# JuanDuGit/DH3D

Measured on AMD Instinct MI355X. Metric: point-clouds/sec, higher is better.
Workload: dtype f32; 1 GPU; local-descriptor forward (basic_config), N=8192 K=8, batch=8; clouds_per_gpu=8, clouds_total=8, points=8192, knn=8, parallelism=clouds sharded over 1 GPU(s), no data-path collective, weights=random-init (no checkpoint blobs exist upstream), steps_in_flight=4

## Files before the change

dh3d_amd/csrc/knn.hip:

```cpp
#include <float.h>
#include <limits.h>

#include <type_traits>

#include "common.h"
#include "wave_ops.h"

#pragma clang fp contract(off)

namespace {

typedef float f32x2 __attribute__((ext_vector_type(2)));
typedef unsigned long long u64;

constexpr int kQueriesPerBlock = 256;
constexpr int kChunk = 1024;
constexpr int kQueue = 16;

struct KnnLadder {
  int log2ct;
  int ctmask;
  int cv;
};

static KnnLadder knn_ladder(int N) {
  int t, v;
  if (N <= 32) { t = 32; v = 1; }
  else if (N <= 64) { t = 64; v = 1; }
  else if (N <= 128) { t = 128; v = 1; }
  else if (N <= 256) { t = 128; v = 2; }
  else if (N <= 512) { t = 128; v = 4; }
  else if (N <= 1024) { t = 256; v = 4; }
  else if (N <= 2048) { t = 256; v = 8; }
  else if (N <= 4096) { t = 512; v = 8; }
  else if (N <= 8192) { t = 1024; v = 8; }
  else { t = 1024; v = (N + 1023) / 1024; }
  KnnLadder l;
  l.ctmask = t - 1;
  l.cv = v;
  l.log2ct = 0;
  while ((1 << l.log2ct) < t) ++l.log2ct;
  return l;
}

__device__ __forceinline__ int cand_slot(int c, int comp) {
  const int g = c >> 2, r = c & 3;
  const int off = (r < 2) ? (2 * comp + r) : (4 + 2 * comp + r);
  return g * 12 + off;
}

__device__ __forceinline__ float knn_bcast(float v, int lane) {
  return __int_as_float(__builtin_amdgcn_readlane(__float_as_int(v), lane));
}

__device__ __forceinline__ int knn_pick_near(unsigned long long m, int gl) {
  const unsigned long long up = m >> gl, dn = m & ((1ull << gl) - 1);
  const int da = up ? __builtin_ctzll(up) : 128;
  const int db = dn ? gl - (63 - __builtin_clzll(dn)) : 128;
  return da <= db ? gl + da : gl - db;
}

template <int KMAX>
struct KnnState {
  u64 keys[KMAX];
  float bound;
};

template <int KMAX, bool KEEP_MIN = false>
__device__ __forceinline__ void knn_insert_key(KnnState<KMAX> &st, const u64 key) {
  if (key < st.keys[KMAX - 1]) {
    if constexpr (KMAX <= 16) {
      bool lt[KMAX];
#pragma unroll
      for (int i = 0; i < KMAX - 1; ++i) lt[i] = key < st.keys[i];
      lt[KMAX - 1] = true;
#pragma unroll
      for (int i = KMAX - 1; i > 0; --i) {
        const u64 in = lt[i - 1] ? st.keys[i - 1] : key;
        st.keys[i] = lt[i] ? in : st.keys[i];
      }
      st.keys[0] = lt[0] ? key : st.keys[0];
    } else {
      st.keys[KMAX - 1] = key;
#pragma unroll
      for (int i = KMAX - 1; i > 0; --i) {
        const u64 a = st.keys[i - 1], b = st.keys[i];
        const bool lt = b < a;
        st.keys[i - 1] = lt ? b : a;
        st.keys[i] = lt ? a : b;
      }
    }
    const unsigned hb = (unsigned)(st.keys[KMAX - 1] >> 32);
    if (hb <= 0x7f800000u) {
      const float dk = __uint_as_float(hb);
      const float nb = __fmul_rn(__fmul_rn(dk, dk), 1.000001f);
      st.bound = KEEP_MIN ? fminf(st.bound, nb) : nb;
    }
  }
}
template <int KMAX, bool KEEP_MIN = false>
__device__ __forceinline__ void knn_offer(KnnState<KMAX> &st, float s, int x, const KnnLadder &lad) {
  if (s <= st.bound) {
    const float d = sqrtf(s);
    const unsigned tb = (unsigned)((x & lad.ctmask) * lad.cv + (x >> lad.log2ct));
    knn_insert_key<KMAX, KEEP_MIN>(st, ((u64)__float_as_uint(d) << 32) | tb);
  }
}


__device__ __forceinline__ void knn_dist8(const float *g0, const f32x2 qx2, const f32x2 qy2, const f32x2 qz2,
                                          f32x2 (&s)[4]) {
  const f32x4 a0 = *reinterpret_cast<const f32x4 *>(g0), a1 = *reinterpret_cast<const f32x4 *>(g0 + 4),
              a2 = *reinterpret_cast<const f32x4 *>(g0 + 8), b0 = *reinterpret_cast<const f32x4 *>(g0 + 12),
              b1 = *reinterpret_cast<const f32x4 *>(g0 + 16), b2 = *reinterpret_cast<const f32x4 *>(g0 + 20);
  {
    const f32x2 dx = f32x2{a0[0], a0[1]} - qx2, dy = f32x2{a0[2], a0[3]} - qy2, dz = f32x2{a1[0], a1[1]} - qz2;
    s[0] = __builtin_elementwise_fma(dz, dz, __builtin_elementwise_fma(dy, dy, dx * dx));
  }
  {
    const f32x2 dx = f32x2{a1[2], a1[3]} - qx2, dy = f32x2{a2[0], a2[1]} - qy2, dz = f32x2{a2[2], a2[3]} - qz2;
    s[1] = __builtin_elementwise_fma(dz, dz, __builtin_elementwise_fma(dy, dy, dx * dx));
  }
  {
    const f32x2 dx = f32x2{b0[0], b0[1]} - qx2, dy = f32x2{b0[2], b0[3]} - qy2, dz = f32x2{b1[0], b1[1]} - qz2;
    s[2] = __builtin_elementwise_fma(dz, dz, __builtin_elementwise_fma(dy, dy, dx * dx));
  }
  {
    const f32x2 dx = f32x2{b1[2], b1[3]} - qx2, dy = f32x2{b2[0], b2[1]} - qy2, dz = f32x2{b2[2], b2[3]} - qz2;
    s[3] = __builtin_elementwise_fma(dz, dz, __builtin_elementwise_fma(dy, dy, dx * dx));
  }
}
__device__ __forceinline__ float knn_min8(const f32x2 (&s)[4]) {
  return fminf(fminf(fminf(s[0][0], s[0][1]), fminf(s[1][0], s[1][1])),
               fminf(fminf(s[2][0], s[2][1]), fminf(s[3][0], s[3][1])));
}

template <int KMAX, bool XYZ_LAYOUT>
__global__ __launch_bounds__(kQueriesPerBlock) void knn_kernel(const float *__restrict__ pos, int N,
                                                              int K, KnnLadder lad,
                                                              int32_t *__restrict__ nn,
                                                              float *__restrict__ dist) {
  __shared__ __attribute__((aligned(16))) float s_c[kChunk * 3];
  __shared__ uint2 s_q[kQueue * kQueriesPerBlock];
  const int b = blockIdx.y;
  const int tid = threadIdx.x;
  const int y = blockIdx.x * kQueriesPerBlock + tid;
  const float *pc = pos + (size_t)b * 3 * N;

  float qx = 0.f, qy = 0.f, qz = 0.f;
  if (y < N) {
    if (XYZ_LAYOUT) { qx = pc[(size_t)y * 3]; qy = pc[(size_t)y * 3 + 1]; qz = pc[(size_t)y * 3 + 2]; }
    else { qx = pc[y]; qy = pc[(size_t)N + y]; qz = pc[(size_t)2 * N + y]; }
  }
  const f32x2 qx2 = {qx, qx}, qy2 = {qy, qy}, qz2 = {qz, qz};

  KnnState<KMAX> st;
#pragma unroll
  for (int i = 0; i < KMAX; ++i) st.keys[i] = ~0ull;
  st.bound = INFINITY;
  int cnt = 0;

  for (int base = 0; base < N; base += kChunk) {
    const int len = min(kChunk, N - base);
    const int len8 = (len + 31) & ~31;
    __syncthreads();
    if (XYZ_LAYOUT) {
      for (int e = tid; e < len8 * 3; e += kQueriesPerBlock) {
        const int c = e / 3, comp = e - c * 3;
        s_c[cand_slot(c, comp)] = c < len ? pc[(size_t)base * 3 + e] : INFINITY;
      }
    } else {
      for (int e = tid; e < len8 * 3; e += kQueriesPerBlock) {
        const int comp = e / len8, c = e - comp * len8;
        s_c[cand_slot(c, comp)] = c < len ? pc[(size_t)comp * N + base + c] : INFINITY;
      }
    }
    __syncthreads();
    const int len32 = (len8 + 31) & ~31;
    for (int j = 0; j < len32; j += 32) {
      f32x2 s[4][4];
      float mn[4];
#pragma unroll
      for (int u = 0; u < 4; ++u) {
        knn_dist8(s_c + ((j >> 2) + 2 * u) * 12, qx2, qy2, qz2, s[u]);
        mn[u] = knn_min8(s[u]);
      }
      const float m = fminf(fminf(mn[0], mn[1]), fminf(mn[2], mn[3]));
      if (__any(y < N && m <= st.bound)) {
#pragma unroll
        for (int u = 0; u < 4; ++u) {
          if (y < N && mn[u] <= st.bound) {
#pragma unroll
            for (int t = 0; t < 8; ++t) {
              const float sv = s[u][t >> 1][t & 1];
              const int x = base + j + 8 * u + t;
              if (sv <= st.bound && x < N) {
                s_q[cnt * kQueriesPerBlock + tid] = make_uint2(__float_as_uint(sv), (unsigned)x);
                ++cnt;
              }
            }
          }
          if (__any(cnt > kQueue - 8)) {
            for (int i = 0; i < kQueue; ++i) {
              if (!__any(i < cnt)) break;
              if (i < cnt) {
                const uint2 e = s_q[i * kQueriesPerBlock + tid];
                knn_offer<KMAX>(st, __uint_as_float(e.x), (int)e.y, lad);
              }
            }
            cnt = 0;
          }
        }
      }
    }
  }
  for (int i = 0; i < kQueue; ++i) {
    if (i < cnt) {
      const uint2 e = s_q[i * kQueriesPerBlock + tid];
      knn_offer<KMAX>(st, __uint_as_float(e.x), (int)e.y, lad);
    }
  }

  if (y < N) {
    int32_t *o_nn = nn + ((size_t)b * N + y) * K;
    float *o_d = dist + ((size_t)b * N + y) * K;
#pragma unroll
    for (int i = 0; i < KMAX; ++i) {
      if (i < K) {
        const unsigned tb = (unsigned)st.keys[i];
        if (st.keys[i] == ~0ull) {
          o_nn[i] = -1;
          o_d[i] = FLT_MAX;
        } else {
          o_nn[i] = (int)(((tb % (unsigned)lad.cv) << lad.log2ct) + tb / (unsigned)lad.cv);
          o_d[i] = __uint_as_float((unsigned)(st.keys[i] >> 32));
        }
      }
    }
  }
}

constexpr int kSortedWaves = 4;
constexpr int kCellInts = 4112;
constexpr int kCellFlag = 4106;

template <int KMAX>
__global__ __launch_bounds__(64 * kSortedWaves) void knn_sorted_kernel(const float4 *__restrict__ sorted,
                                                                    const float *__restrict__ gbox, int N,
                                                                    int K, KnnLadder lad,
                                                                    int32_t *__restrict__ nn,
                                                                    float *__restrict__ dist, const int *__restrict__ gate) {
  if (gate && !gate[(size_t)blockIdx.y * kCellInts + kCellFlag]) return;
  __shared__ __attribute__((aligned(16))) float s_c[kSortedWaves][64 * 3];
  __shared__ uint2 s_q[kSortedWaves][kQueue * 64];
  __shared__ int s_id[kSortedWaves][64];
  const int b = blockIdx.y;
  const int lane = threadIdx.x & 63, wave = threadIdx.x >> 6;
  const int NG = (N + 63) / 64;
  const int g = blockIdx.x * kSortedWaves + wave;
  if (g >= NG) return;
  const float4 *sc = sorted + (size_t)b * N;
  const float4 *gb = reinterpret_cast<const float4 *>(gbox) + (size_t)b * NG * 2;
  float *my_c = s_c[wave];
  uint2 *my_q = s_q[wave];
  int *my_id = s_id[wave];

  const int qi = g * 64 + lane;
  const bool valid = qi < N;
  const float4 pad = make_float4(INFINITY, INFINITY, INFINITY, __int_as_float(-1));
  float4 qr = valid ? sc[qi] : pad;
  const f32x2 qx2 = {qr.x, qr.x}, qy2 = {qr.y, qr.y}, qz2 = {qr.z, qr.z};
  const float4 qlo = gb[g * 2], qhi = gb[g * 2 + 1];

  KnnState<KMAX> st;
#pragma unroll
  for (int i = 0; i < KMAX; ++i) st.keys[i] = ~0ull;
  st.bound = INFINITY;
  int cnt = 0;
  float wave_bound = INFINITY;

  auto drain = [&]() {
    const int deepest = -wave_min_i32(-cnt);
    uint2 nxt = my_q[lane];
#pragma unroll 1
    for (int i = 0; i < deepest; ++i) {
      const uint2 e = nxt;
      if (i + 1 < deepest) nxt = my_q[(i + 1) * 64 + lane];
      if (i < cnt) knn_offer<KMAX>(st, __uint_as_float(e.x), (int)e.y, lad);
    }
    cnt = 0;
    wave_bound = wave_max_f32(valid ? st.bound : 0.f);
  };

  auto scan_group = [&](int gcc, const float4 cr) {
    my_c[cand_slot(lane, 0)] = cr.x;
    my_c[cand_slot(lane, 1)] = cr.y;
    my_c[cand_slot(lane, 2)] = cr.z;
    my_id[lane] = __float_as_int(cr.w);
    __builtin_amdgcn_wave_barrier();
    const int clen = min(64, N - gcc * 64);
    for (int j = 0; j < clen; j += 32) {
      f32x2 s[4][4];
      float mn[4];
#pragma unroll
      for (int u = 0; u < 4; ++u) {
        knn_dist8(my_c + ((j >> 2) + 2 * u) * 12, qx2, qy2, qz2, s[u]);
        mn[u] = knn_min8(s[u]);
      }
      const float m = fminf(fminf(mn[0], mn[1]), fminf(mn[2], mn[3]));
      if (__any(valid && m <= st.bound)) {
#pragma unroll
        for (int u = 0; u < 4; ++u) {
          if (valid && mn[u] <= st.bound) {
#pragma unroll
            for (int t = 0; t < 8; ++t) {
              const float sv = s[u][t >> 1][t & 1];
              if (sv <= st.bound && j + 8 * u + t < clen) {
                my_q[cnt * 64 + lane] = make_uint2(__float_as_uint(sv), (unsigned)my_id[j + 8 * u + t]);
                ++cnt;
              }
            }
          }
          if (__any(cnt > kQueue - 8)) drain();
        }
      }
    }
    __builtin_amdgcn_wave_barrier();
  };
  auto load_group = [&](int gcc) { const int ci = gcc * 64 + lane; return ci < N ? sc[ci] : pad; };

  scan_group(g, qr);
  if (__any(cnt > 0)) drain();

  const int cg = g >> 6, NC = (NG + 63) >> 6;
  for (int tier = 0; tier < 2; ++tier) {
    for (int k = 0; k < 2 * NC; ++k) {
      const int ci = cg + ((k & 1) ? (k + 1) / 2 : -(k / 2));
      if (ci < 0 || ci >= NC) continue;
      const int c0 = ci * 64, gl = min(max(g - c0, 0), 63);
      const int gi = c0 + lane;
      const bool other = gi < NG && gi != g;
      float bd = INFINITY;
      float4 clo = make_float4(INFINITY, INFINITY, INFINITY, 0.f), chi = clo;
      if (other) {
        clo = gb[gi * 2];
        chi = gb[gi * 2 + 1];
        const float ex = fmaxf(fmaxf(clo.x - qhi.x, qlo.x - chi.x), 0.f);
        const float ey = fmaxf(fmaxf(clo.y - qhi.y, qlo.y - chi.y), 0.f);
        const float ez = fmaxf(fmaxf(clo.z - qhi.z, qlo.z - chi.z), 0.f);
        bd = (ex * ex + ey * ey + ez * ez) * 0.99999f;
      }
      unsigned long long mask =
          tier == 0 ? __ballot(other && bd == 0.f) : __ballot(other && bd > 0.f && bd <= wave_bound);
      if (!mask) continue;
      int l = knn_pick_near(mask, gl);
      mask &= ~(1ull << l);
      float4 nxt = load_group(c0 + l);
      while (true) {
        const int lcur = l;
        const float4 cr = nxt;
        const bool more = mask != 0;
        if (more) {
          l = knn_pick_near(mask, gl);
          mask &= ~(1ull << l);
          nxt = load_group(c0 + l);
        }
        const float bdl = __int_as_float(__builtin_amdgcn_readlane(__float_as_int(bd), lcur));
        if (bdl <= wave_bound) {
          const float lx = knn_bcast(clo.x, lcur), ly = knn_bcast(clo.y, lcur), lz = knn_bcast(clo.z, lcur);
          const float hx = knn_bcast(chi.x, lcur), hy = knn_bcast(chi.y, lcur), hz = knn_bcast(chi.z, lcur);
          const float px = fmaxf(fmaxf(lx - qr.x, qr.x - hx), 0.f);
          const float py = fmaxf(fmaxf(ly - qr.y, qr.y - hy), 0.f);
          const float pz = fmaxf(fmaxf(lz - qr.z, qr.z - hz), 0.f);
          const float pd = (px * px + py * py + pz * pz) * 0.99999f;
          if (__any(valid && pd <= st.bound)) scan_group(c0 + lcur, cr);
        }
        if (!more) break;
      }
    }
  }
  if (__any(cnt > 0)) drain();

  if (valid) {
    const int y = __float_as_int(qr.w);
    int32_t *o_nn = nn + ((size_t)b * N + y) * K;
    float *o_d = dist + ((size_t)b * N + y) * K;
#pragma unroll
    for (int i = 0; i < KMAX; ++i) {
      if (i < K) {
        const unsigned tb = (unsigned)st.keys[i];
        if (st.keys[i] == ~0ull) {
          o_nn[i] = -1;
          o_d[i] = FLT_MAX;
        } else {
          o_nn[i] = (int)(((tb % (unsigned)lad.cv) << lad.log2ct) + tb / (unsigned)lad.cv);
          o_d[i] = __uint_as_float((unsigned)(st.keys[i] >> 32));
        }
      }
    }
  }
}

template <int S>
__host__ __device__ constexpr int knn_split_lds_bytes() {
  return S * (64 * 3 * 4 + kQueue * 64 * 8 + 64 * 4 + 64 * 4 + 64 * 4);
}
template <int KMAX, int S>
__device__ __forceinline__ void knn_split_body(const float4 *__restrict__ sorted, const float *__restrict__ gbox, int N, int K,
                                               const KnnLadder lad, int32_t *__restrict__ nn, float *__restrict__ dist,
                                               const int b, const int g, unsigned char *lds, const int wave0 = 0) {
  static_assert(KMAX * 64 * sizeof(u64) <= kQueue * 64 * sizeof(uint2), "a K-list fits its wave's survivor queue");
  uint2 (*s_q)[kQueue * 64] = reinterpret_cast<uint2 (*)[kQueue * 64]>(lds);
  float (*s_c)[64 * 3] = reinterpret_cast<float (*)[64 * 3]>(lds + S * kQueue * 64 * 8);
  int (*s_id)[64] = reinterpret_cast<int (*)[64]>(lds + S * (kQueue * 64 * 8 + 64 * 3 * 4));
  float (*s_share)[64] = reinterpret_cast<float (*)[64]>(lds + S * (kQueue * 64 * 8 + 64 * 3 * 4 + 64 * 4));
  float (*s_kth)[64] = reinterpret_cast<float (*)[64]>(lds + S * (kQueue * 64 * 8 + 64 * 3 * 4 + 64 * 8));
  constexpr int R = (KMAX + S - 1) / S - 1;
  const int lane = threadIdx.x & 63;
  const int wave = __builtin_amdgcn_readfirstlane((int)(threadIdx.x >> 6) - wave0);
  const int NG = (N + 63) / 64;
  const float4 *sc = sorted + (size_t)b * N;
  const float4 *gb = reinterpret_cast<const float4 *>(gbox) + (size_t)b * NG * 2;
  float *my_c = s_c[wave];
  uint2 *my_q = s_q[wave];
  int *my_id = s_id[wave];

  const int qi = g * 64 + lane;
  const bool valid = qi < N;
  const float4 pad = make_float4(INFINITY, INFINITY, INFINITY, __int_as_float(-1));
  const float4 qr = valid ? sc[qi] : pad;
  const f32x2 qx2 = {qr.x, qr.x}, qy2 = {qr.y, qr.y}, qz2 = {qr.z, qr.z};
  const float4 qlo = gb[g * 2], qhi = gb[g * 2 + 1];

  KnnState<KMAX> st;
#pragma unroll
  for (int i = 0; i < KMAX; ++i) st.keys[i] = ~0ull;
  st.bound = INFINITY;
  int cnt = 0;
  float wave_bound = INFINITY;
  s_share[wave][lane] = INFINITY;
  s_kth[wave][lane] = INFINITY;
  __syncthreads();

  auto adopt = [&](float mx) {
    float mk = st.bound;
#pragma unroll
    for (int w = 1; w < S; ++w) {
      mx = fmaxf(mx, s_share[(wave + w) % S][lane]);
      mk = fminf(mk, s_kth[(wave + w) % S][lane]);
    }
    st.bound = fminf(mk, mx);
    wave_bound = wave_max_f32(valid ? st.bound : 0.f);
  };

  auto drain = [&]() {
    const int deepest = -wave_min_i32(-cnt);
    uint2 nxt = my_q[lane];
#pragma unroll 1
    for (int i = 0; i < deepest; ++i) {
      const uint2 e = nxt;
      if (i + 1 < deepest) nxt = my_q[(i + 1) * 64 + lane];
      if (i < cnt) knn_offer<KMAX, true>(st, __uint_as_float(e.x), (int)e.y, lad);
    }
    cnt = 0;
    const unsigned hb = (unsigned)(st.keys[R] >> 32);
    float mx = INFINITY;
    if (hb <= 0x7f800000u) {
      const float dr = __uint_as_float(hb);
      mx = __fmul_rn(__fmul_rn(dr, dr), 1.000001f);
    }
    s_share[wave][lane] = mx;
    const unsigned hk = (unsigned)(st.keys[KMAX - 1] >> 32);
    if (hk <= 0x7f800000u) {
      const float dk = __uint_as_float(hk);
      s_kth[wave][lane] = __fmul_rn(__fmul_rn(dk, dk), 1.000001f);
    }
    adopt(mx);
  };

  auto scan_group = [&](int gcc, const float4 cr) {
    my_c[cand_slot(lane, 0)] = cr.x;
    my_c[cand_slot(lane, 1)] = cr.y;
    my_c[cand_slot(lane, 2)] = cr.z;
    my_id[lane] = __float_as_int(cr.w);
    __builtin_amdgcn_wave_barrier();
    const int clen = min(64, N - gcc * 64);
    for (int j = 0; j < clen; j += 32) {
      f32x2 sq[4][4];
      float mn[4];
#pragma unroll
      for (int u = 0; u < 4; ++u) {
        knn_dist8(my_c + ((j >> 2) + 2 * u) * 12, qx2, qy2, qz2, sq[u]);
        mn[u] = knn_min8(sq[u]);
      }
      const float m = fminf(fminf(mn[0], mn[1]), fminf(mn[2], mn[3]));
      if (__any(valid && m <= st.bound)) {
#pragma unroll
        for (int u = 0; u < 4; ++u) {
          if (valid && mn[u] <= st.bound) {
#pragma unroll
            for (int t = 0; t < 8; ++t) {
              const float sv = sq[u][t >> 1][t & 1];
              if (sv <= st.bound && j + 8 * u + t < clen) {
                my_q[cnt * 64 + lane] = make_uint2(__float_as_uint(sv), (unsigned)my_id[j + 8 * u + t]);
                ++cnt;
              }
            }
          }
          if (__any(cnt > kQueue - 8)) drain();
        }
      }
    }
    __builtin_amdgcn_wave_barrier();
  };
  auto load_group = [&](int gcc) { const int ci = gcc * 64 + lane; return ci < N ? sc[ci] : pad; };

  const int NO = (NG - wave + S - 1) / S, NCH = (NO + 63) >> 6;
  const int jg = g / S, cj = min(jg >> 6, max(NCH - 1, 0));
  bool other = false;
  float bd = INFINITY;
  float4 clo = make_float4(INFINITY, INFINITY, INFINITY, 0.f), chi = clo;
  auto fetch_boxes = [&](int ci) {
    const int j = ci * 64 + lane, gi = j * S + wave;
    other = j < NO && gi != g;
    if (other) {
      clo = gb[gi * 2];
      chi = gb[gi * 2 + 1];
    }
  };
  auto test_boxes = [&]() {
    bd = INFINITY;
    if (other) {
      const float ex = fmaxf(fmaxf(clo.x - qhi.x, qlo.x - chi.x), 0.f);
      const float ey = fmaxf(fmaxf(clo.y - qhi.y, qlo.y - chi.y), 0.f);
      const float ez = fmaxf(fmaxf(clo.z - qhi.z, qlo.z - chi.z), 0.f);
      bd = (ex * ex + ey * ey + ez * ez) * 0.99999f;
    }
  };
  if (NCH == 1) fetch_boxes(0);

  {
    my_c[cand_slot(lane, 0)] = qr.x;
    my_c[cand_slot(lane, 1)] = qr.y;
    my_c[cand_slot(lane, 2)] = qr.z;
    my_id[lane] = __float_as_int(qr.w);
    __builtin_amdgcn_wave_barrier();
    const int clen = min(64, N - g * 64);
    for (int blk = wave; blk * 8 < clen; blk += S) {
      f32x2 sq[4];
      knn_dist8(my_c + 2 * blk * 12, qx2, qy2, qz2, sq);
      if (valid) {
#pragma unroll
        for (int t = 0; t < 8; ++t) {
          const float sv = sq[t >> 1][t & 1];
          if (sv <= st.bound && blk * 8 + t < clen) {
            my_q[cnt * 64 + lane] = make_uint2(__float_as_uint(sv), (unsigned)my_id[blk * 8 + t]);
            ++cnt;
          }
        }
      }
      if (__any(cnt > 0)) drain();
    }
    __builtin_amdgcn_wave_barrier();
    __syncthreads();
    adopt(s_share[wave][lane]);
  }
  for (int tier = 0; tier < 2; ++tier) {
    for (int k = 0; k < 2 * NCH; ++k) {
      const int ci = cj + ((k & 1) ? (k + 1) / 2 : -(k / 2));
      if (ci < 0 || ci >= NCH) continue;
      if (NCH > 1) fetch_boxes(ci);
      if (NCH > 1 || tier == 0) test_boxes();
      const int gl = min(max(jg - ci * 64, 0), 63);
      if (tier == 1) adopt(s_share[wave][lane]);
      unsigned long long mask =
          tier == 0 ? __ballot(other && bd == 0.f) : __ballot(other && bd > 0.f && bd <= wave_bound);
      if (!mask) continue;
      int l = knn_pick_near(mask, gl);
      mask &= ~(1ull << l);
      float4 nxt = load_group((ci * 64 + l) * S + wave);
      while (true) {
        const int lcur = l;
        const float4 cr = nxt;
        const bool more = mask != 0;
        if (more) {
          l = knn_pick_near(mask, gl);
          mask &= ~(1ull << l);
          nxt = load_group((ci * 64 + l) * S + wave);
        }
        const float bdl = knn_bcast(bd, lcur);
        if (bdl <= wave_bound) {
          const float lx = knn_bcast(clo.x, lcur), ly = knn_bcast(clo.y, lcur), lz = knn_bcast(clo.z, lcur);
          const float hx = knn_bcast(chi.x, lcur), hy = knn_bcast(chi.y, lcur), hz = knn_bcast(chi.z, lcur);
          const float px = fmaxf(fmaxf(lx - qr.x, qr.x - hx), 0.f);
          const float py = fmaxf(fmaxf(ly - qr.y, qr.y - hy), 0.f);
          const float pz = fmaxf(fmaxf(lz - qr.z, qr.z - hz), 0.f);
          const float pd = (px * px + py * py + pz * pz) * 0.99999f;
          if (__any(valid && pd <= st.bound)) scan_group((ci * 64 + lcur) * S + wave, cr);
        }
        if (!more) break;
      }
    }
  }
  if (__any(cnt > 0)) drain();

  for (int step = S / 2; step >= 1; step >>= 1) {
    __syncthreads();
    if (wave >= step && wave < 2 * step) {
#pragma unroll
      for (int i = 0; i < KMAX; ++i)
        my_q[i * 64 + lane] = make_uint2((unsigned)st.keys[i], (unsigned)(st.keys[i] >> 32));
    }
    __syncthreads();
    if (wave < step) {
      const uint2 *oq = s_q[wave + step];
#pragma unroll
      for (int i = 0; i < KMAX; ++i) {
        const uint2 e = oq[i * 64 + lane];
        const u64 key = ((u64)e.y << 32) | e.x;
        if (key < st.keys[KMAX - 1]) {
          st.keys[KMAX - 1] = key;
#pragma unroll
          for (int t = KMAX - 1; t > 0; --t) {
            const u64 a = st.keys[t - 1], c = st.keys[t];
            const bool lt = c < a;
            st.keys[t - 1] = lt ? c : a;
            st.keys[t] = lt ? a : c;
          }
        }
      }
    }
  }

  if (wave == 0 && valid) {
    const int y = __float_as_int(qr.w);
    int32_t *o_nn = nn + ((size_t)b * N + y) * K;
    float *o_d = dist + ((size_t)b * N + y) * K;
#pragma unroll
    for (int i = 0; i < KMAX; ++i) {
      if (i < K) {
        const unsigned tb = (unsigned)st.keys[i];
        if (st.keys[i] == ~0ull) {
          o_nn[i] = -1;
          o_d[i] = FLT_MAX;
        } else {
          o_nn[i] = (int)(((tb % (unsigned)lad.cv) << lad.log2ct) + tb / (unsigned)lad.cv);
          o_d[i] = __uint_as_float((unsigned)(st.keys[i] >> 32));
        }
      }
    }
  }
}


template <int KMAX, int S>
__global__ __launch_bounds__(64 * S) void knn_split_kernel(const float4 *__restrict__ sorted,
                                                         const float *__restrict__ gbox, int N, int K,
                                                         KnnLadder lad, int32_t *__restrict__ nn,
                                                         float *__restrict__ dist, const int *__restrict__ gate) {
  if (gate && !gate[(size_t)blockIdx.y * kCellInts + kCellFlag]) return;
  __shared__ __attribute__((aligned(16))) unsigned char s_lds[knn_split_lds_bytes<S>()];
  const unsigned ng = (unsigned)((N + 63) / 64);
  knn_split_body<KMAX, S>(sorted, gbox, N, K, lad, nn, dist, blockIdx.y, (int)((blockIdx.x + 37u * blockIdx.y) % ng), s_lds);
}

template <int CPL, bool XYZ>
__global__ __launch_bounds__(256) void knn_small_kernel(const float *__restrict__ pos, int N, int K, KnnLadder lad,
                                                       int32_t *__restrict__ nn, float *__restrict__ dist, int Q) {
  const int b = blockIdx.y, lane = threadIdx.x & 63;
  const int wave = __builtin_amdgcn_readfirstlane(threadIdx.x >> 6);
  const int q0 = (blockIdx.x * 4 + wave) * Q;
  if (q0 >= N) return;
  const float *base = pos + (size_t)b * N * 3;
  float cx[CPL], cy[CPL], cz[CPL];
  unsigned tbk[CPL];
#pragma unroll
  for (int c = 0; c < CPL; ++c) {
    const int j = lane + 64 * c, jj = j < N ? j : 0;
    cx[c] = XYZ ? base[(size_t)jj * 3] : base[jj];
    cy[c] = XYZ ? base[(size_t)jj * 3 + 1] : base[(size_t)N + jj];
    cz[c] = XYZ ? base[(size_t)jj * 3 + 2] : base[(size_t)2 * N + jj];
    tbk[c] = j < N ? (unsigned)((j & lad.ctmask) * lad.cv + (j >> lad.log2ct)) : 0xFFFFFFFFu;
  }
#pragma unroll 1
  for (int qi = 0; qi < Q; ++qi) {
    const int q = q0 + qi;
    if (q >= N) break;
    const float qx = XYZ ? base[(size_t)q * 3] : base[q];
    const float qy = XYZ ? base[(size_t)q * 3 + 1] : base[(size_t)N + q];
    const float qz = XYZ ? base[(size_t)q * 3 + 2] : base[(size_t)2 * N + q];
    unsigned kd[CPL];
#pragma unroll
    for (int c = 0; c < CPL; ++c) {
      const float dx = qx - cx[c], dy = qy - cy[c], dz = qz - cz[c];
      const float d = sqrtf(__builtin_fmaf(dz, dz, __builtin_fmaf(dy, dy, dx * dx)));
      kd[c] = tbk[c] != 0xFFFFFFFFu ? __float_as_uint(d) : 0xFFFFFFFFu;
    }
    u64 need = 0;
    unsigned my_hi = 0xFFFFFFFFu, my_lo = 0xFFFFFFFFu;
    u64 m1 = ~0ull, m2 = ~0ull;
    bool more = false;
    auto rescan = [&]() {
      m1 = ~0ull; m2 = ~0ull;
      int cnt = 0;
#pragma unroll
      for (int c = 0; c < CPL; ++c) {
        const u64 key = ((u64)kd[c] << 32) | tbk[c];
        const bool ok = key >= need && key != ~0ull;
        const bool c1 = ok && key < m1, c2 = ok && key < m2;
        m2 = c1 ? m1 : (c2 ? key : m2);
        m1 = c1 ? key : m1;
        cnt += ok ? 1 : 0;
      }
      more = cnt > 2;
    };
    rescan();
    for (int r = 0; r < K; ++r) {
      const unsigned hi = wave_min_u32((unsigned)(m1 >> 32));
      const unsigned lo = wave_min_u32((unsigned)(m1 >> 32) == hi ? (unsigned)m1 : 0xFFFFFFFFu);
      if (lane == r) { my_hi = hi; my_lo = lo; }
      const u64 sel = ((u64)hi << 32) | lo;
      if (sel == ~0ull) break;
      need = sel + 1;
      const bool won = m1 == sel;
      const bool dry = won && m2 == ~0ull && more;
      m1 = won ? m2 : m1;
      m2 = won ? ~0ull : m2;
      if (__ballot(dry) != 0ull) rescan();
    }
    if (lane < K) {
      const size_t o = ((size_t)b * N + q) * K + lane;
      if (my_hi == 0xFFFFFFFFu && my_lo == 0xFFFFFFFFu) {
        nn[o] = -1;
        dist[o] = FLT_MAX;
      } else {
        nn[o] = (int)(((my_lo % (unsigned)lad.cv) << lad.log2ct) + my_lo / (unsigned)lad.cv);
        dist[o] = __uint_as_float(my_hi);
      }
    }
  }
}

template <bool XYZ>
int knn_launch(const float *pos, int B, int N, int K, int32_t *nn, float *dist, hipStream_t s) {
  const KnnLadder lad = knn_ladder(N);
  if (N <= 2048) {
    const int Q = (long long)B * N <= 16384 ? 2 : 4;
    dim3 sgrid(dh3d_cdiv(N, 4 * Q), B), sblock(256);
    if (N <= 512) hipLaunchKernelGGL((knn_small_kernel<8, XYZ>), sgrid, sblock, 0, s, pos, N, K, lad, nn, dist, Q);
    else if (N <= 1024) hipLaunchKernelGGL((knn_small_kernel<16, XYZ>), sgrid, sblock, 0, s, pos, N, K, lad, nn, dist, Q);
    else hipLaunchKernelGGL((knn_small_kernel<32, XYZ>), sgrid, sblock, 0, s, pos, N, K, lad, nn, dist, Q);
    return dh3d_launch_status();
  }
  dim3 grid(dh3d_cdiv(N, kQueriesPerBlock), B), block(kQueriesPerBlock);
  if (K <= 4) hipLaunchKernelGGL((knn_kernel<4, XYZ>), grid, block, 0, s, pos, N, K, lad, nn, dist);
  else if (K <= 8) hipLaunchKernelGGL((knn_kernel<8, XYZ>), grid, block, 0, s, pos, N, K, lad, nn, dist);
  else if (K <= 16) hipLaunchKernelGGL((knn_kernel<16, XYZ>), grid, block, 0, s, pos, N, K, lad, nn, dist);
  else if (K <= 32) hipLaunchKernelGGL((knn_kernel<32, XYZ>), grid, block, 0, s, pos, N, K, lad, nn, dist);
  else hipLaunchKernelGGL((knn_kernel<64, XYZ>), grid, block, 0, s, pos, N, K, lad, nn, dist);
  return dh3d_launch_status();
}

template <int KMAX>
__global__ __launch_bounds__(256) void knn_anydp_kernel(const float *__restrict__ pos, int Dp, int N, int K, KnnLadder lad,
                                                        int32_t *__restrict__ nn, float *__restrict__ dist) {
  __shared__ float s_c[16][256];
  const int b = blockIdx.y, y = blockIdx.x * 256 + threadIdx.x;
  const float *pc = pos + (size_t)b * Dp * N;
  float q[16];
#pragma unroll
  for (int dp = 0; dp < 16; ++dp) q[dp] = (dp < Dp && y < N) ? pc[(size_t)dp * N + y] : 0.f;
  u64 keys[KMAX];
#pragma unroll
  for (int i = 0; i < KMAX; ++i) keys[i] = ~0ull;
  for (int x0 = 0; x0 < N; x0 += 256) {
    __syncthreads();
    for (int dp = 0; dp < Dp; ++dp) s_c[dp][threadIdx.x] = x0 + (int)threadIdx.x < N ? pc[(size_t)dp * N + x0 + threadIdx.x] : 0.f;
    __syncthreads();
    const int cnt = min(256, N - x0);
    for (int j = 0; j < cnt; ++j) {
      float sum = 0.f;
      for (int dp = 0; dp < Dp; ++dp) {
        const float val = s_c[dp][j] - q[dp];
        sum = __builtin_fmaf(val, val, sum);
      }
      const float d = sqrtf(sum);
      const int x = x0 + j;
      const unsigned tb = (unsigned)((x & lad.ctmask) * lad.cv + (x >> lad.log2ct));
      const u64 key = ((u64)__float_as_uint(d) << 32) | tb;
      if (key < keys[K - 1]) {
        int i = K - 1;
        while (i > 0 && keys[i - 1] > key) { keys[i] = keys[i - 1]; --i; }
        keys[i] = key;
      }
    }
  }
  if (y >= N) return;
  int32_t *o_nn = nn + ((size_t)b * N + y) * K;
  float *o_d = dist + ((size_t)b * N + y) * K;
  for (int i = 0; i < K; ++i) {
    if (keys[i] == ~0ull) { o_nn[i] = -1; o_d[i] = 3.402823466e+38f; continue; }
    const unsigned tb = (unsigned)keys[i];
    o_nn[i] = (int)(((tb % (unsigned)lad.cv) << lad.log2ct) + tb / (unsigned)lad.cv);
    o_d[i] = __uint_as_float((unsigned)(keys[i] >> 32));
  }
}

}

DH3D_API int dh3d_knn_bruteforce(const float *positions, int B, int Dp, int N, int K, int32_t *nn,
                                 float *dist, void *stream) {
  DH3D_REQUIRE(positions && nn && dist && B > 0 && N > 0 && K > 0 && Dp > 0);
  DH3D_SUPPORTED(K <= 64 && B <= 65535);
  if (Dp == 3) return knn_launch<false>(positions, B, N, K, nn, dist, (hipStream_t)stream);
  DH3D_SUPPORTED(Dp <= 16);
  const KnnLadder lad = knn_ladder(N);
  dim3 grid(dh3d_cdiv(N, 256), B), block(256);
  hipStream_t s = (hipStream_t)stream;
  if (K <= 8) hipLaunchKernelGGL(knn_anydp_kernel<8>, grid, block, 0, s, positions, Dp, N, K, lad, nn, dist);
  else if (K <= 16) hipLaunchKernelGGL(knn_anydp_kernel<16>, grid, block, 0, s, positions, Dp, N, K, lad, nn, dist);
  else hipLaunchKernelGGL(knn_anydp_kernel<64>, grid, block, 0, s, positions, Dp, N, K, lad, nn, dist);
  return dh3d_launch_status();
}

DH3D_API int dh3d_knn_bruteforce_xyz(const float *xyz, int B, int N, int K, int32_t *nn, float *dist,
                                     void *stream) {
  DH3D_REQUIRE(xyz && nn && dist && B > 0 && N > 0 && K > 0);
  DH3D_SUPPORTED(K <= 64 && B <= 65535);
  return knn_launch<true>(xyz, B, N, K, nn, dist, (hipStream_t)stream);
}

static int knn_sorted_launch(const float *sorted, const float *gbox, int B, int N, int K, int32_t *nn, float *dist,
                             const int *gate, void *stream) {
  DH3D_REQUIRE(sorted && gbox && nn && dist && B > 0 && N > 0 && K > 0);
  DH3D_SUPPORTED(K <= 64 && B <= 65535);
  const KnnLadder lad = knn_ladder(N);
  const int NG = (N + 63) / 64;
  dim3 grid(dh3d_cdiv(NG, kSortedWaves), B), block(64 * kSortedWaves);
  hipStream_t s = (hipStream_t)stream;
  const float4 *so = reinterpret_cast<const float4 *>(sorted);
  const long long groups = (long long)NG * B;
  const int S = groups <= 256 ? 8 : groups <= 1280 ? 4 : groups <= 4096 ? 2 : 0;
  if (S > 0 && K <= 16) {
    dim3 sgrid(NG, B);
#define DH3D_SPLIT_CASE(KM, SS)                                                                               \
  if (K <= KM && S == SS) {                                                                                  \
    hipLaunchKernelGGL((knn_split_kernel<KM, SS>), sgrid, dim3(64 * SS), 0, s, so, gbox, N, K, lad, nn, dist, gate); \
    return dh3d_launch_status();                                                                             \
  }
    DH3D_SPLIT_CASE(4, 2) DH3D_SPLIT_CASE(4, 4)
    DH3D_SPLIT_CASE(8, 2) DH3D_SPLIT_CASE(8, 4) DH3D_SPLIT_CASE(8, 8)
    DH3D_SPLIT_CASE(16, 2) DH3D_SPLIT_CASE(16, 4) DH3D_SPLIT_CASE(16, 8)
#undef DH3D_SPLIT_CASE
  }
  if (K <= 4) hipLaunchKernelGGL((knn_sorted_kernel<4>), grid, block, 0, s, so, gbox, N, K, lad, nn, dist, gate);
  else if (K <= 8) hipLaunchKernelGGL((knn_sorted_kernel<8>), grid, block, 0, s, so, gbox, N, K, lad, nn, dist, gate);
  else if (K <= 16) hipLaunchKernelGGL((knn_sorted_kernel<16>), grid, block, 0, s, so, gbox, N, K, lad, nn, dist, gate);
  else if (K <= 32) hipLaunchKernelGGL((knn_sorted_kernel<32>), grid, block, 0, s, so, gbox, N, K, lad, nn, dist, gate);
  else hipLaunchKernelGGL((knn_sorted_kernel<64>), grid, block, 0, s, so, gbox, N, K, lad, nn, dist, gate);
  return dh3d_launch_status();
}

DH3D_API int dh3d_knn_sorted(const float *sorted, const float *gbox, int B, int N, int K, int32_t *nn,
                             float *dist, void *stream) {
  return knn_sorted_launch(sorted, gbox, B, N, K, nn, dist, nullptr, stream);
}

constexpr int kGridCap = 256;

__device__ __forceinline__ unsigned knn_spread4(unsigned v) {
  return (v & 1u) | ((v & 2u) << 2) | ((v & 4u) << 4) | ((v & 8u) << 6);
}
__device__ __forceinline__ void knn_cswap(u64 &a, u64 &b) {
  const bool lt = b < a;
  const u64 lo = lt ? b : a, hi = lt ? a : b;
  a = lo; b = hi;
}
template <int CTRL>
__device__ __forceinline__ u64 knn_dpp_u64(u64 v) {
  const int lo = __builtin_amdgcn_update_dpp(0, (int)(unsigned)v, CTRL, 0xF, 0xF, true);
  const int hi = __builtin_amdgcn_update_dpp(0, (int)(unsigned)(v >> 32), CTRL, 0xF, 0xF, true);
  return ((u64)(unsigned)hi << 32) | (unsigned)lo;
}
template <int CTRL>
__device__ __forceinline__ void knn_merge_step(KnnState<8> &st) {
  u64 c[8];
#pragma unroll
  for (int i = 0; i < 8; ++i) {
    const u64 mine = st.keys[i], theirs = knn_dpp_u64<CTRL>(st.keys[7 - i]);
    c[i] = mine < theirs ? mine : theirs;
  }
  knn_cswap(c[0], c[4]); knn_cswap(c[1], c[5]); knn_cswap(c[2], c[6]); knn_cswap(c[3], c[7]);
  knn_cswap(c[0], c[2]); knn_cswap(c[1], c[3]); knn_cswap(c[4], c[6]); knn_cswap(c[5], c[7]);
  knn_cswap(c[0], c[1]); knn_cswap(c[2], c[3]); knn_cswap(c[4], c[5]); knn_cswap(c[6], c[7]);
#pragma unroll
  for (int i = 0; i < 8; ++i) st.keys[i] = c[i];
}
template <int L>
__device__ __forceinline__ void knn_merge_sublanes(KnnState<8> &st) {
  if (L >= 2) knn_merge_step<0xB1>(st);
  if (L >= 4) knn_merge_step<0x4E>(st);
  if (L >= 8) knn_merge_step<0x141>(st);
  const unsigned hb = (unsigned)(st.keys[7] >> 32);
  if (hb <= 0x7f800000u) {
    const float dk = __uint_as_float(hb);
    st.bound = __fmul_rn(__fmul_rn(dk, dk), 1.000001f);
  }
}

template <int L, int SF>
__global__ __launch_bounds__(256) void knn_grid_kernel(const float4 *__restrict__ sorted, const float *__restrict__ gbox,
                                                      const int *__restrict__ cells, int N, int K, int D, KnnLadder lad,
                                                      int32_t *__restrict__ nn, float *__restrict__ dist) {
  constexpr int QB = 256 / L;
  static_assert(SF == 0 || (L == 4 && SF <= 4), "the merged scan: 64 queries per workgroup, at most four waves");
  constexpr int kGridLds = 3 * 64 * 4 + QB * kGridCap * 2 + QB * 4;
  constexpr int kSplitLds = SF == 2 ? 2 * knn_split_lds_bytes<2>() : SF > 0 ? knn_split_lds_bytes<(SF > 0 ? SF : 1)>() : 0;
  __shared__ __attribute__((aligned(16))) unsigned char s_raw[kGridLds > kSplitLds ? kGridLds : kSplitLds];
  const int b = blockIdx.y, lane = threadIdx.x & 63, sub = lane & (L - 1);
  if (cells[(size_t)b * kCellInts + kCellFlag]) {
    if constexpr (SF > 0) {
      const int ngq = (N + 63) / 64;
      if constexpr (SF == 2) {
        const int half = (int)(threadIdx.x >> 7), pairs = (ngq + 1) / 2;
        if ((int)blockIdx.x >= pairs) return;
        const int g0 = (int)blockIdx.x + half * pairs;
        if (g0 >= ngq) return;
        knn_split_body<8, 2>(sorted, gbox, N, K, lad, nn, dist, b, (int)(((unsigned)g0 + 37u * (unsigned)b) % (unsigned)ngq),
                             s_raw + half * knn_split_lds_bytes<2>(), half * 2);
      } else if (threadIdx.x < 64 * SF) {
        knn_split_body<8, (SF > 0 ? SF : 1)>(sorted, gbox, N, K, lad, nn, dist, b, (int)((blockIdx.x + 37u * (unsigned)b) % (unsigned)ngq), s_raw);
      }
    }
    return;
  }
  const int qi = (int)((blockIdx.x + 37u * (unsigned)b) % gridDim.x) * QB + threadIdx.x / L;
  const bool valid = qi < N;
  const float4 *sc = sorted + (size_t)b * N;
  const int *ct = cells + (size_t)b * kCellInts;
  const float *hd = reinterpret_cast<const float *>(ct) + 4100;
  const float lo[3] = {hd[0], hd[1], hd[2]}, scl[3] = {hd[3], hd[4], hd[5]};
  const float4 qr = sc[valid ? qi : N - 1];
  const float q[3] = {qr.x, qr.y, qr.z};
  const unsigned sched = (unsigned)ct[4107];
  int nb[3] = {0, 0, 0}, drop[3] = {0, 0, 0};
#pragma unroll
  for (int s = 0; s < 12; ++s) {
    const int a = (int)((sched >> (2 * s)) & 3u);
#pragma unroll
    for (int c = 0; c < 3; ++c) {
      nb[c] += (int)(a == c);
      drop[c] += (int)(a == c && s >= 12 - D);
    }
  }
  const int span = 1 << D;
  int cq[3], gmax[3];
  float w[3], eps[3];
#pragma unroll
  for (int a = 0; a < 3; ++a) {
    cq[a] = min((4 << nb[a]) - 1, max(0, (int)((q[a] - lo[a]) * scl[a]))) >> (2 + drop[a]);
    gmax[a] = ((1 << nb[a]) >> drop[a]) - 1;
    w[a] = (float)(4 << drop[a]) / scl[a];
    eps[a] = 2.5e-6f * ((float)(4 << nb[a]) / scl[a]);
  }
  unsigned (*s_ctab)[64] = reinterpret_cast<unsigned (*)[64]>(s_raw);
  if (threadIdx.x < 192) {
    const int a = threadIdx.x >> 6, v = threadIdx.x & 63;
    unsigned code = 0;
    int rem = nb[a] - drop[a];
    for (int s = 0; s < 12 - D; ++s)
      if ((int)((sched >> (2 * s)) & 3u) == a && rem > 0) {
        --rem;
        code |= (unsigned)((v >> rem) & 1) << (11 - s);
      }
    s_ctab[a][v] = code;
  }
  __syncthreads();
  auto cell_code = [&](int ax, int ay, int az) { return s_ctab[0][ax & 63] | s_ctab[1][ay & 63] | s_ctab[2][az & 63]; };
  KnnState<8> st;
#pragma unroll
  for (int i = 0; i < 8; ++i) st.keys[i] = ~0ull;
  st.bound = valid ? INFINITY : -1.f;

  auto axis_d2 = [&](int a, int o) {
    const float l = lo[a] + (float)(cq[a] + o) * w[a];
    const float d = fmaxf(fmaxf(fmaxf(l - q[a], q[a] - (l + w[a])), 0.f) - eps[a], 0.f);
    return d * d;
  };
  float d2x[5];
  unsigned bitx[5];
  bool okx[5];
#pragma unroll
  for (int t = 0; t < 5; ++t) {
    const int ax = cq[0] + t - 2;
    okx[t] = (unsigned)ax <= (unsigned)gmax[0];
    d2x[t] = okx[t] ? axis_d2(0, t - 2) : INFINITY;
    bitx[t] = s_ctab[0][ax & 63];
  }
  auto inside = [&](int R) {
    float G = INFINITY;
#pragma unroll
    for (int a = 0; a < 3; ++a) {
      if (cq[a] - R > 0) G = fminf(G, (q[a] - (lo[a] + (float)(cq[a] - R) * w[a])) - eps[a]);
      if (cq[a] + R < gmax[a]) G = fminf(G, ((lo[a] + (float)(cq[a] + R + 1) * w[a]) - q[a]) - eps[a]);
    }
    if (G == INFINITY) return true;
    G = fmaxf(G, 0.f);
    return st.bound < G * G * 0.99999f;
  };

  auto keep_one_copy = [&]() {
    if (sub != 0) {
#pragma unroll
      for (int i = 0; i < 8; ++i) st.keys[i] = ~0ull;
    }
  };
  unsigned short (*s_list)[kGridCap] = reinterpret_cast<unsigned short (*)[kGridCap]>(s_raw + 3 * 64 * 4);
  int *s_cnt = reinterpret_cast<int *>(s_raw + 3 * 64 * 4 + QB * kGridCap * 2);
  const int qs = threadIdx.x / L;
  auto direct = [&](int j) {
    const float4 r = sc[j];
    const float dx = r.x - q[0], dy = r.y - q[1], dz = r.z - q[2];
    knn_offer<8, false>(st, fmaf(dz, dz, fmaf(dy, dy, dx * dx)), __float_as_int(r.w), lad);
  };
  auto enqueue = [&](int beg, int end) {
    const int len = end - beg;
    if (len <= 0) return;
    const int off = atomicAdd(&s_cnt[qs], len);
    const int fit = min(len, kGridCap - off);
    for (int k = 0; k < fit; ++k) s_list[qs][off + k] = (unsigned short)(beg + k);
    for (int k = max(fit, 0); k < len; ++k) direct(beg + k);
  };
  auto drain = [&]() {
    __builtin_amdgcn_fence(__ATOMIC_SEQ_CST, "wavefront");
    __builtin_amdgcn_wave_barrier();
    const int total = min(s_cnt[qs], kGridCap);
#pragma unroll 1
    for (int base = sub; base < total; base += 4 * L) {
      float4 r[4];
      bool ok[4];
#pragma unroll
      for (int u = 0; u < 4; ++u) {
        const int i = base + u * L;
        ok[u] = i < total;
        r[u] = sc[s_list[qs][min(i, total - 1)]];
      }
#pragma unroll
      for (int u = 0; u < 4; ++u) {
        const float dx = r[u].x - q[0], dy = r[u].y - q[1], dz = r[u].z - q[2];
        const float s2 = fmaf(dz, dz, fmaf(dy, dy, dx * dx));
        knn_offer<8, false>(st, ok[u] ? s2 : __builtin_nanf(""), __float_as_int(r[u].w), lad);
      }
    }
    __builtin_amdgcn_fence(__ATOMIC_SEQ_CST, "wavefront");
    __builtin_amdgcn_wave_barrier();
  };
  auto column = [&](auto tmask, int dy, int dz) __attribute__((always_inline)) {
    constexpr int TMASK = decltype(tmask)::value;
    const int ay = cq[1] + dy - 2, az = cq[2] + dz - 2;
    if ((unsigned)ay > (unsigned)gmax[1] || (unsigned)az > (unsigned)gmax[2]) return;
    const float d2yz = axis_d2(1, dy - 2) + axis_d2(2, dz - 2);
    const unsigned bityz = cell_code(0, ay, az);
    int beg[5], end[5];
#pragma unroll
    for (int t = 0; t < 5; ++t)
      if (TMASK >> t & 1) {
        beg[t] = ct[bityz | bitx[t]];
        end[t] = ct[(bityz | bitx[t]) + span];
      }
    if constexpr (TMASK != 0b01110) {
#pragma unroll
      for (int t = 0; t < 5; ++t)
        if (TMASK >> t & 1) {
          if (!okx[t] || (d2yz + d2x[t]) * 0.99999f > st.bound) continue;
          enqueue(beg[t], end[t]);
        }
    } else {
      int len[5], tot = 0;
#pragma unroll
      for (int t = 0; t < 5; ++t)
        if (TMASK >> t & 1) {
          len[t] = okx[t] && !((d2yz + d2x[t]) * 0.99999f > st.bound) ? end[t] - beg[t] : 0;
          tot += len[t];
        }
      if (tot == 0) return;
      int off = atomicAdd(&s_cnt[qs], tot);
#pragma unroll
      for (int t = 0; t < 5; ++t)
        if (TMASK >> t & 1) {
          const int fit = min(len[t], kGridCap - off);
          unsigned short *dst = &s_list[qs][off];
#pragma unroll
          for (int k = 0; k < 4; ++k)
            if (k < fit) dst[k] = (unsigned short)(beg[t] + k);
          for (int k = 4; k < fit; ++k) dst[k] = (unsigned short)(beg[t] + k);
          for (int k = max(fit, 0); k < len[t]; ++k) direct(beg[t] + k);
          off += len[t];
        }
    }
  };
  auto begin_pass = [&]() __attribute__((always_inline)) {
    if (sub == 0) s_cnt[qs] = 0;
    __builtin_amdgcn_fence(__ATOMIC_SEQ_CST, "wavefront");
    __builtin_amdgcn_wave_barrier();
  };
  begin_pass();
#pragma unroll 1
  for (int ci = sub; ci < 9; ci += L) column(std::integral_constant<int, 0b01110>{}, 1 + ci % 3, 1 + ci / 3);
  drain();
  knn_merge_sublanes<L>(st);
  keep_one_copy();
  begin_pass();
  bool exact = false;
  int ylo = -2, zlo = -2, ny = 5, ncol = valid ? 25 : 0;
  if (valid && st.bound < INFINITY) {
    const float r = sqrtf(st.bound) * 1.0001f;
    int dlo[3], dhi[3];
#pragma unroll
    for (int a = 0; a < 3; ++a) {
      const float inv = scl[a] / (float)(4 << drop[a]);
      dlo[a] = min(0, max(0, (int)floorf((q[a] - r - eps[a] - lo[a]) * inv)) - cq[a]);
      dhi[a] = max(0, min(gmax[a], (int)floorf((q[a] + r + eps[a] - lo[a]) * inv)) - cq[a]);
    }
    const int by = dhi[1] - dlo[1] + 1, bc = by * (dhi[2] - dlo[2] + 1);
    if (dlo[0] >= -2 && dhi[0] <= 2 && bc <= 128) {
      exact = true;
      ylo = dlo[1]; zlo = dlo[2]; ny = by; ncol = bc;
    }
  }
#pragma unroll 1
  for (int ci = sub; ci < ncol; ci += L) {
    const int iz = ci / ny, dy = ylo + (ci - iz * ny), dz = zlo + iz;
    if (abs(dy) <= 1 && abs(dz) <= 1) column(std::integral_constant<int, 0b10001>{}, dy + 2, dz + 2);
    else column(std::integral_constant<int, 0b11111>{}, dy + 2, dz + 2);
  }
  drain();
  knn_merge_sublanes<L>(st);
  const bool done = !valid || exact || inside(2);
  if (__any(!done)) {
    if (done) {
      keep_one_copy();
    } else {
#pragma unroll
      for (int i = 0; i < 8; ++i) st.keys[i] = ~0ull;
      const int NG = (N + 63) >> 6;
      const float4 *gb = reinterpret_cast<const float4 *>(gbox) + (size_t)b * NG * 2;
#pragma unroll 1
      for (int g = sub; g < NG; g += L) {
        const float4 lo4 = gb[2 * g], hi4 = gb[2 * g + 1];
        const float ex = fmaxf(fmaxf(lo4.x - q[0], q[0] - hi4.x), 0.f), ey = fmaxf(fmaxf(lo4.y - q[1], q[1] - hi4.y), 0.f),
                    ez = fmaxf(fmaxf(lo4.z - q[2], q[2] - hi4.z), 0.f);
        if ((ex * ex + ey * ey + ez * ez) * 0.99999f > st.bound) continue;
        const int j1 = min(N, g * 64 + 64);
#pragma unroll 1
        for (int j = g * 64; j < j1; j += 8) {
          float4 r8[8];
#pragma unroll
          for (int u = 0; u < 8; ++u) r8[u] = sc[min(j + u, j1 - 1)];
#pragma unroll
          for (int u = 0; u < 8; ++u) {
            const float dx = r8[u].x - q[0], dy = r8[u].y - q[1], dz = r8[u].z - q[2];
            const float s2 = fmaf(dz, dz, fmaf(dy, dy, dx * dx));
            knn_offer<8, false>(st, j + u < j1 ? s2 : __builtin_nanf(""), __float_as_int(r8[u].w), lad);
          }
        }
      }
    }
    knn_merge_sublanes<L>(st);
  }
  if (valid) {
    const int y = __float_as_int(qr.w);
#pragma unroll
    for (int e = 0; e < 8 / L; ++e) {
      const int slot = e * L + sub;
      if (slot >= K) break;
      u64 key = st.keys[0];
#pragma unroll
      for (int i = 1; i < 8; ++i) key = slot == i ? st.keys[i] : key;
      const size_t o = ((size_t)b * N + y) * K + slot;
      if (key == ~0ull) {
        nn[o] = -1;
        dist[o] = FLT_MAX;
      } else {
        const unsigned tb = (unsigned)key;
        nn[o] = (int)(((tb % (unsigned)lad.cv) << lad.log2ct) + tb / (unsigned)lad.cv);
        dist[o] = __uint_as_float((unsigned)(key >> 32));
      }
    }
  }
}

constexpr int kGridLanes = 4;

struct KnnGridPlan {
  int sf, drop;
};
static KnnGridPlan knn_grid_plan(int B, int N) {
  KnnGridPlan p{0, 0};
  while (p.drop < 6 && ((long long)N << p.drop) <= 3072) ++p.drop;
  const long long groups = (long long)((N + 63) / 64) * B;
  if (kGridLanes == 4 && groups <= 4096) p.sf = groups > 1280 ? 2 : 4;
  return p;
}

DH3D_API int dh3d_knn_grid_plan(int B, int N, int K) {
  if (B <= 0 || N <= 0 || K <= 0 || K > 8 || N > 16384 || B > 65535) return -1;
  const KnnGridPlan p = knn_grid_plan(B, N);
  return p.sf + 16 * p.drop;
}

DH3D_API int dh3d_knn_grid(const float *sorted, const float *gbox, const int32_t *cells, int B, int N, int K, int32_t *nn,
                           float *dist, void *stream) {
  DH3D_REQUIRE(sorted && gbox && cells && nn && dist && B > 0 && N > 0 && K > 0);
  DH3D_SUPPORTED(K <= 8 && N <= 16384 && B <= 65535);
  const KnnLadder lad = knn_ladder(N);
  constexpr int kLanes = kGridLanes;
  const KnnGridPlan plan = knn_grid_plan(B, N);
  const int D = plan.drop;
  const dim3 grid(dh3d_cdiv(N, 256 / kLanes), B);
  const float4 *so = reinterpret_cast<const float4 *>(sorted);
  if (plan.sf == 2) {
    hipLaunchKernelGGL((knn_grid_kernel<4, 2>), grid, dim3(256), 0, (hipStream_t)stream, so, gbox, cells, N, K, D, lad, nn, dist);
    return dh3d_launch_status();
  }
  if (plan.sf == 4) {
    hipLaunchKernelGGL((knn_grid_kernel<4, 4>), grid, dim3(256), 0, (hipStream_t)stream, so, gbox, cells, N, K, D, lad, nn, dist);
    return dh3d_launch_status();
  }
  hipLaunchKernelGGL((knn_grid_kernel<kLanes, 0>), grid, dim3(256), 0, (hipStream_t)stream, so, gbox, cells, N, K, D, lad, nn, dist);
  if (dh3d_launch_status() != DH3D_OK) return DH3D_ERR_LAUNCH;
  return knn_sorted_launch(sorted, gbox, B, N, K, nn, dist, cells, stream);
}
```

Before: 38490 point-clouds/sec.

## Cache the workgroup's cell-range window in LDS and hoist grid constants

The workgroup computes the bounding box of its queries' grid cells and preloads each cell's begin offset and length, packed into 32 bits, into an LDS window. Column lookups then read that window instead of making two global loads per cell into the cell table. Per-axis grid constants are now computed once by a single thread, shared through LDS and made wave-uniform with readfirstlane, instead of every thread recomputing them. The cost is extra LDS, two more barriers, and a preload that may fetch cells no query uses; the 15-bit packing assumes offsets and counts fit, which holds for N=8192.

```diff
diff --git a/dh3d_amd/csrc/knn.hip b/dh3d_amd/csrc/knn.hip
--- a/dh3d_amd/csrc/knn.hip
+++ b/dh3d_amd/csrc/knn.hip
@@ -867,6 +867,7 @@
 }
 
 constexpr int kGridCap = 256;
+constexpr int kGridWin = 1536;
 
 __device__ __forceinline__ unsigned knn_spread4(unsigned v) {
   return (v & 1u) | ((v & 2u) << 2) | ((v & 4u) << 4) | ((v & 8u) << 6);
@@ -914,7 +915,10 @@
                                                       int32_t *__restrict__ nn, float *__restrict__ dist) {
   constexpr int QB = 256 / L;
   static_assert(SF == 0 || (L == 4 && SF <= 4), "the merged scan: 64 queries per workgroup, at most four waves");
-  constexpr int kGridLds = 3 * 64 * 4 + QB * kGridCap * 2 + QB * 4;
+  constexpr int kGcOff = 3 * 64 * 4 + QB * kGridCap * 2 + QB * 4;
+  constexpr int kWinOff = kGcOff + 32 * 4;
+  constexpr int kGridLds = kWinOff + kGridWin * 4;
+  static_assert(kGridLds <= 40960, "four workgroups share a CU's 160 KB");
   constexpr int kSplitLds = SF == 2 ? 2 * knn_split_lds_bytes<2>() : SF > 0 ? knn_split_lds_bytes<(SF > 0 ? SF : 1)>() : 0;
   __shared__ __attribute__((aligned(16))) unsigned char s_raw[kGridLds > kSplitLds ? kGridLds : kSplitLds];
   const int b = blockIdx.y, lane = threadIdx.x & 63, sub = lane & (L - 1);
@@ -939,43 +943,92 @@
   const float4 *sc = sorted + (size_t)b * N;
   const int *ct = cells + (size_t)b * kCellInts;
   const float *hd = reinterpret_cast<const float *>(ct) + 4100;
-  const float lo[3] = {hd[0], hd[1], hd[2]}, scl[3] = {hd[3], hd[4], hd[5]};
+  const float lo[3] = {hd[0], hd[1], hd[2]};
   const float4 qr = sc[valid ? qi : N - 1];
   const float q[3] = {qr.x, qr.y, qr.z};
   const unsigned sched = (unsigned)ct[4107];
-  int nb[3] = {0, 0, 0}, drop[3] = {0, 0, 0};
-#pragma unroll
-  for (int s = 0; s < 12; ++s) {
-    const int a = (int)((sched >> (2 * s)) & 3u);
-#pragma unroll
-    for (int c = 0; c < 3; ++c) {
-      nb[c] += (int)(a == c);
-      drop[c] += (int)(a == c && s >= 12 - D);
-    }
-  }
   const int span = 1 << D;
-  int cq[3], gmax[3];
-  float w[3], eps[3];
-#pragma unroll
-  for (int a = 0; a < 3; ++a) {
-    cq[a] = min((4 << nb[a]) - 1, max(0, (int)((q[a] - lo[a]) * scl[a]))) >> (2 + drop[a]);
-    gmax[a] = ((1 << nb[a]) >> drop[a]) - 1;
-    w[a] = (float)(4 << drop[a]) / scl[a];
-    eps[a] = 2.5e-6f * ((float)(4 << nb[a]) / scl[a]);
-  }
   unsigned (*s_ctab)[64] = reinterpret_cast<unsigned (*)[64]>(s_raw);
+  int *s_gc = reinterpret_cast<int *>(s_raw + kGcOff);
   if (threadIdx.x < 192) {
     const int a = threadIdx.x >> 6, v = threadIdx.x & 63;
     unsigned code = 0;
-    int rem = nb[a] - drop[a];
-    for (int s = 0; s < 12 - D; ++s)
-      if ((int)((sched >> (2 * s)) & 3u) == a && rem > 0) {
-        --rem;
-        code |= (unsigned)((v >> rem) & 1) << (11 - s);
+    int bit = 0;
+    for (int s = 11 - D; s >= 0; --s)
+      if ((int)((sched >> (2 * s)) & 3u) == a) {
+        code |= (unsigned)((v >> bit) & 1) << (11 - s);
+        ++bit;
       }
     s_ctab[a][v] = code;
+  } else if (threadIdx.x == 192) {
+    const float scl[3] = {hd[3], hd[4], hd[5]};
+    int nb[3] = {0, 0, 0}, drop[3] = {0, 0, 0};
+#pragma unroll
+    for (int s = 0; s < 12; ++s) {
+      const int a = (int)((sched >> (2 * s)) & 3u);
+#pragma unroll
+      for (int c = 0; c < 3; ++c) {
+        nb[c] += (int)(a == c);
+        drop[c] += (int)(a == c && s >= 12 - D);
+      }
+    }
+#pragma unroll
+    for (int a = 0; a < 3; ++a) {
+      s_gc[a] = (4 << nb[a]) - 1;
+      s_gc[3 + a] = 2 + drop[a];
+      s_gc[6 + a] = ((1 << nb[a]) >> drop[a]) - 1;
+      s_gc[9 + a] = __float_as_int((float)(4 << drop[a]) / scl[a]);
+      s_gc[12 + a] = __float_as_int(2.5e-6f * ((float)(4 << nb[a]) / scl[a]));
+      s_gc[15 + a] = __float_as_int(scl[a] / (float)(4 << drop[a]));
+      s_gc[18 + a] = 64;
+      s_gc[21 + a] = -1;
+    }
   }
   __syncthreads();
+  int cq[3], gmax[3];
+  float w[3], eps[3], cpu[3];
+#pragma unroll
+  for (int a = 0; a < 3; ++a) {
+    const int qmax = __builtin_amdgcn_readfirstlane(s_gc[a]), sh = __builtin_amdgcn_readfirstlane(s_gc[3 + a]);
+    cq[a] = min(qmax, max(0, (int)((q[a] - lo[a]) * hd[3 + a]))) >> sh;
+    gmax[a] = __builtin_amdgcn_readfirstlane(s_gc[6 + a]);
+    w[a] = __int_as_float(__builtin_amdgcn_readfirstlane(s_gc[9 + a]));
+    eps[a] = __int_as_float(__builtin_amdgcn_readfirstlane(s_gc[12 + a]));
+    cpu[a] = __int_as_float(__builtin_amdgcn_readfirstlane(s_gc[15 + a]));
+  }
+  if (sub == 0) {
+#pragma unroll
+    for (int a = 0; a < 3; ++a) {
+      atomicMin(&s_gc[18 + a], cq[a]);
+      atomicMax(&s_gc[21 + a], cq[a]);
+    }
+  }
+  __syncthreads();
+  unsigned *s_win = reinterpret_cast<unsigned *>(s_raw + kWinOff);
+  const int wx0 = __builtin_amdgcn_readfirstlane(s_gc[18]) - 2;
+  const int wnx = __builtin_amdgcn_readfirstlane(s_gc[21]) + 3 - wx0;
+  const int wy0 = max(0, __builtin_amdgcn_readfirstlane(s_gc[19]) - 2);
+  const int wny = min(gmax[1], __builtin_amdgcn_readfirstlane(s_gc[22]) + 2) + 1 - wy0;
+  const int wz0 = max(0, __builtin_amdgcn_readfirstlane(s_gc[20]) - 2);
+  const int wnz = min(gmax[2], __builtin_amdgcn_readfirstlane(s_gc[23]) + 2) + 1 - wz0;
+  const int wcells = wnx * wny * wnz;
+  const bool win = wcells <= kGridWin;
+  if (win) {
+    const float rnx = 1.f / (float)wnx, rny = 1.f / (float)wny;
+    for (int i = threadIdx.x; i < wcells; i += 256) {
+      const int row = (int)(((float)i + 0.5f) * rnx), z = (int)(((float)row + 0.5f) * rny);
+      const int ax = wx0 + (i - row * wnx), ay = wy0 + (row - z * wny), az = wz0 + z;
+      unsigned v = 0;
+      if ((unsigned)ax <= (unsigned)gmax[0]) {
+        const unsigned code = s_ctab[0][ax] | s_ctab[1][ay] | s_ctab[2][az];
+        const int beg = ct[code];
+        v = (unsigned)beg | (unsigned)(ct[code + span] - beg) << 15;
+      }
+      s_win[i] = v;
+    }
+  }
+  __syncthreads();
+  const int wxq = cq[0] - 2 - wx0;
   auto cell_code = [&](int ax, int ay, int az) { return s_ctab[0][ax & 63] | s_ctab[1][ay & 63] | s_ctab[2][az & 63]; };
   KnnState<8> st;
 #pragma unroll
@@ -1060,14 +1113,25 @@
     const int ay = cq[1] + dy - 2, az = cq[2] + dz - 2;
     if ((unsigned)ay > (unsigned)gmax[1] || (unsigned)az > (unsigned)gmax[2]) return;
     const float d2yz = axis_d2(1, dy - 2) + axis_d2(2, dz - 2);
-    const unsigned bityz = cell_code(0, ay, az);
     int beg[5], end[5];
-#pragma unroll
-    for (int t = 0; t < 5; ++t)
-      if (TMASK >> t & 1) {
-        beg[t] = ct[bityz | bitx[t]];
-        end[t] = ct[(bityz | bitx[t]) + span];
-      }
+    if (win && (unsigned)(ay - wy0) < (unsigned)wny && (unsigned)(az - wz0) < (unsigned)wnz) {
+      const unsigned *wr = s_win + ((az - wz0) * wny + (ay - wy0)) * wnx + wxq;
+#pragma unroll
+      for (int t = 0; t < 5; ++t)
+        if (TMASK >> t & 1) {
+          const unsigned v = wr[t];
+          beg[t] = (int)(v & 0x7fffu);
+          end[t] = beg[t] + (int)(v >> 15);
+        }
+    } else {
+      const unsigned bityz = cell_code(0, ay, az);
+#pragma unroll
+      for (int t = 0; t < 5; ++t)
+        if (TMASK >> t & 1) {
+          beg[t] = ct[bityz | bitx[t]];
+          end[t] = ct[(bityz | bitx[t]) + span];
+        }
+    }
     if constexpr (TMASK != 0b01110) {
 #pragma unroll
       for (int t = 0; t < 5; ++t)
@@ -1118,7 +1182,7 @@
     int dlo[3], dhi[3];
 #pragma unroll
     for (int a = 0; a < 3; ++a) {
-      const float inv = scl[a] / (float)(4 << drop[a]);
+      const float inv = cpu[a];
       dlo[a] = min(0, max(0, (int)floorf((q[a] - r - eps[a] - lo[a]) * inv)) - cq[a]);
       dhi[a] = max(0, min(gmax[a], (int)floorf((q[a] + r + eps[a] - lo[a]) * inv)) - cq[a]);
     }
```

After: 37680 point-clouds/sec. 0.979x the previous value.
